# manycore-research/faceformer

Measured on AMD Instinct MI355X. Metric: decoded edges/sec (greedy face-loop decode, pointer selections/s), 256-edge wireframes, higher is better.
Workload: dtype f32; 1 GPU; BASELINE config 2: configs/ours.yml model.num_lines=256: 1 synthetic 256-edge wireframe(s) per GPU, F=256 anchor sequences x 36 greedy steps, default-xavier synthetic weights; wireframes_per_gpu=1, edges=256, max_face_length=37, decode_steps=36, parallelism=wireframe-sharded x1, RCCL all-gather of predictions

## Files before the change

faceformer_amd/csrc/ff_common.h:

```cpp
#pragma once
#include <hip/hip_runtime.h>
#include <stdint.h>
#include <stdio.h>
#include <string.h>

#include "faceformer_hip.h"

#define FF_WAVE 64
#define FF_MAX_STREAMS 8

typedef float f32x4 __attribute__((ext_vector_type(4)));
typedef float f32x16 __attribute__((ext_vector_type(16)));

void ff_set_error(const char* fmt, ...);

#define FF_CHECK_ARG(cond, ...)           \
  do {                                    \
    if (!(cond)) {                        \
      ff_set_error(__VA_ARGS__);          \
      return FF_ERR_ARG;                  \
    }                                     \
  } while (0)

#define FF_CHECK_HIP(expr)                                                             \
// ... 31 lines not shown
  ~FFProfScope() {
    if (on) ff_prof_close(st);
  }
};

unsigned long long ff_tuning_epoch();
void ff_tuning_changed();

int ff_num_cus();

enum FFKnob {
  FF_K_L0_FOLD = 0,
  FF_K_POINTER_FOLD,
  FF_K_LAST_QKV_ONE_LAUNCH_ROWS,
  FF_K_PINNED_COUNTERS,
  FF_K_DEBUG_TIMING,
  FF_K_DMA_MIN_ROWS, FF_K_DMA_MIN_ROWS_N512, FF_K_DMA_MIN_ROWS_WIDE,
  FF_K_SK_HYBRID, FF_K_SK_HYBRID_FIX, FF_K_SK_HYBRID_MAXLEFT8, FF_K_SK_HYBRID_MINU, FF_K_SK_HYBRID_FORCE,
  FF_K_NO_PANEL,
  FF_K_X3_SMALL_SPLIT,
  FF_K_RK_SPLIT_OLD, FF_K_RK_SPLIT_YOUNG, FF_K_RK_PHASE, FF_K_RK_ROTATE,
  FF_K_X3_NEED_N1024, FF_K_X3_NEED_N512,
  FF_K_X2H_ATTN,
  FF_K_COUNT
};
int ff_knob(int id);

size_t ff_attention_planes_stride();
bool ff_attention_x2h_ok(const ff_attn_desc& d);
int ff_attention_x2h_launch(const ff_attn_desc& d, const void* planes, long long plane_stride, hipStream_t st);

struct ff_pointer_sync {
  int* seen;
  int* arrive;
  int* host_slot;
  int host_which;
  float* next_stats;
  int logits_ready;
  const int* slot;
  int* fin;
  int fin_j, term_lo, term_hi;
};
int ff_pointer_argmax_sync(const float* p, int ldp, const float* memory, int S, int E, const unsigned char* mask,
                           const int* kv_len, const unsigned char* extra_mask, int ldextra, int B, int seqs_per_group,
                           int* next_tok, float* best, float* second, float* logprob, float* logits, int ldlogits,
                           float* next_rows, int ldnext, int* count_ge, int ge_bound, int* count_eq, int eq_value,
// ... 34 lines not shown
int ff_pointer_constrained_ahead_sync(float* logits, int ldlogits, int S, const unsigned char* mask, const int* kv_len, int B,
                                      int seqs_per_group, const unsigned* follows, int L, int flags, int ntok, int term_lo,
                                      int term_hi, const int* fin_in, const int* first_in, const int* prev_in, unsigned* visited,
                                      unsigned char* mask_rows, int* next_tok, float* logprob, int* fin_out, int* dead_end,
                                      int* first_out, int* prev_out, const float* memory, int E, float* next_rows, int ldnext,
                                      float* next_stats, int* count_ge, const unsigned char* close_dist,
                                      const unsigned char* cycle_len, int budget, int* arrive, int* host_slot, ff_stream_t stream);
int ff_constrain_init(int* tok, float* lp, int* fin, int* dead, int* first, int* prev, unsigned* visited, int Bc, int Fc, int f0,
                      const int* num_input, int pad_tok, int term_lo, int term_hi, int ntok, const unsigned* follows, int L,
                      hipStream_t st);
int ff_constrain_finalize(const int* tok, const float* lp, const int* fin, const int* dead, int Btot, int T, const int* steps_dev,
                          const int* num_input, int dedup, int F, int w0, int nw, int Fc, int f0, int b0, int64_t* predict,
                          float* logprob, int* dead_end, int* seq_of_row, hipStream_t st);

int ff_beam_constrained_select_sync(const ff_beam_constrained_step* step, int* arrive, int* host_slot, ff_stream_t stream);
int ff_constrain_beam_init(int* tok, float* score, int* fin, int* dead, int* parent, int* first, int* prev, unsigned* visited, int Bc,
                           int Fc, int W, int f0, const int* num_input, int pad_tok, int term_lo, int term_hi, int ntok,
                           const unsigned* follows, int L, hipStream_t st);
int ff_constrain_beam_dead(const int* dead, int Btot, const int* steps_dev, const int* num_input, int dedup, int F, int W, int w0,
                           int nw, int Fc, int f0, int b0, int* dead_end, hipStream_t st);

int ff_transpose(const float* in, int ld_in, int rows, int cols, float* out, int ld_out, hipStream_t st);

extern "C" __attribute__((visibility("hidden"))) int ff_x3_prepare_stream(hipStream_t st);
int ff_stream_scratch(hipStream_t st, size_t bytes, float** out);

__device__ __forceinline__ float ff_wave_sum(float v) {
#pragma unroll
  for (int off = 32; off > 0; off >>= 1) v += __shfl_xor(v, off, FF_WAVE);
  return v;
}
__device__ __forceinline__ float ff_wave_max(float v) {
#pragma unroll
  for (int off = 32; off > 0; off >>= 1) v = fmaxf(v, __shfl_xor(v, off, FF_WAVE));
  return v;
}

__device__ __forceinline__ float ff_halves_sum(float v) {
  const auto r = __builtin_amdgcn_permlane32_swap(__float_as_uint(v), __float_as_uint(v), false, false);
  return __uint_as_float(r[0]) + __uint_as_float(r[1]);
}
__device__ __forceinline__ float ff_halves_max(float v) {
  const auto r = __builtin_amdgcn_permlane32_swap(__float_as_uint(v), __float_as_uint(v), false, false);
  return fmaxf(__uint_as_float(r[0]), __uint_as_float(r[1]));
}

// ... 8 lines not shown
```

faceformer_amd/csrc/ff_device.h:

```cpp
#pragma once
#include "ff_common.h"

typedef float f32x2 __attribute__((ext_vector_type(2)));

#define FF_GLOBAL __attribute__((address_space(1)))
typedef unsigned long long ff_u64;

__device__ __forceinline__ f32x4 ff_ld16(const float* p) { return *reinterpret_cast<const f32x4*>(p); }
__device__ __forceinline__ f32x2 ff_ld8(const float* p) { return *reinterpret_cast<const f32x2*>(p); }
__device__ __forceinline__ float ff_ld4(const float* p) { return *p; }
__device__ __forceinline__ void ff_st16(float* p, f32x4 v) { *reinterpret_cast<f32x4*>(p) = v; }
__device__ __forceinline__ void ff_st8(float* p, f32x2 v) { *reinterpret_cast<f32x2*>(p) = v; }
__device__ __forceinline__ void ff_st4(float* p, float v) { *p = v; }
__device__ __forceinline__ int ff_ld4i(const int* p) { return *p; }
__device__ __forceinline__ void ff_st4i(int* p, int v) { *p = v; }
__device__ __forceinline__ void ff_store_tile(float* cp, int ldc, int row0, int col, int M, bool colok, const float (&v)[16]) {
  float* p = cp + (size_t)row0 * ldc + col;
  if (row0 - (row0 & 4) + 32 <= M) {
    if (colok) {
#pragma unroll
      for (int e = 0; e < 16; ++e) ff_st4(p + (size_t)((e & 3) + 8 * (e >> 2)) * ldc, v[e]);
    }
  } else {
#pragma unroll
// ... 14 lines not shown
  const float* res;
  float* C;
  int lda, ldw, ldr, ldc;
  int M, N, K;
  int n_split, act;
  int tiles_m, tiles_n;
  long long batch_stride_a, batch_stride_w, batch_stride_c;
  const float* ln_in;
  int ln_nseg;
  float ln_eps;
  const float* rowtab;
  int ld_rowtab, rowtab_div, rowtab_cols;
  float* ln_out;
};

bool ff_gemm_dma_f32_ok(const GemmArgs& a, int batch);
int ff_gemm_dma_f32(const GemmArgs& a, hipStream_t st, int bn = 128);

__device__ __forceinline__ float ff_sum8(float v) {
  v += __builtin_bit_cast(float, __builtin_amdgcn_update_dpp(0, __builtin_bit_cast(int, v), 0xB1, 0xF, 0xF, true));
  v += __builtin_bit_cast(float, __builtin_amdgcn_update_dpp(0, __builtin_bit_cast(int, v), 0x4E, 0xF, 0xF, true));
  v += __builtin_bit_cast(float, __builtin_amdgcn_update_dpp(0, __builtin_bit_cast(int, v), 0x141, 0xF, 0xF, true));
  return v;
}

__host__ __device__ constexpr int ff_gemm_small_lds_floats(int mode, int nw) {
  return nw * 16 * 64 + (mode == 2 ? 32 * 33 : 0) + (mode == 1 ? 64 : 0);
}

template <int KQ, int MODE, int NW>
__device__ __forceinline__ void ff_gemm_small_tile(const GemmArgs& g, int tile, long long bz, float* red) {
  static_assert(NW == 4 || NW == 8, "4 or 8 waves");
  constexpr int RPW = 16 / NW;
  const int tid = threadIdx.x, wave = tid >> 6, lane = tid & 63, half = lane >> 5, l32 = lane & 31;
  const int m0 = (tile / g.tiles_n) * 32, n0 = (tile % g.tiles_n) * 32;
  const float* Asrc = ((g.A2 != nullptr && n0 >= g.n_split) ? g.A2 : g.A) + bz * g.batch_stride_a;
  int row = m0 + l32, col = n0 + l32;
  row = row < g.M ? row : g.M - 1;
  col = col < g.N ? col : g.N - 1;
  const float* ap = Asrc + (size_t)row * g.lda + wave * KQ + half * 4;
  const float* wp = g.W + bz * g.batch_stride_w + (size_t)col * g.ldw + wave * KQ + half * 4;
  constexpr int NG = KQ / 8;
  constexpr int GB = NG < 4 ? NG : 4;
  f32x4 a[2][GB], b[2][GB];
#pragma unroll
  for (int j = 0; j < GB; ++j) {
// ... 709 lines not shown
```

faceformer_amd/csrc/ff_engine.hip:

```cpp
#include <chrono>
#include <cstdlib>
#include <mutex>
#include <vector>

#include "ff_common.h"
#include "ff_device.h"
#include "ff_launch.h"

namespace {

struct Bump {
  char* base;
  size_t size, off;
  bool ok;
  Bump(void* p, size_t n) : base((char*)p), size(n), off(0), ok(true) {}
  template <typename T>
  T* take(size_t count) {
    size_t bytes = ff_align_up(count * sizeof(T), 256);
    if (off + bytes > size) { ok = false; off += bytes; return nullptr; }
    T* r = reinterpret_cast<T*>(base + off);
    off += bytes;
    return r;
  }
};
// ... 112 lines not shown
    return gemm(d.A, d.lda, d.A2, d.n_split, d.W, d.ldw, d.bias, d.res, d.ldr, d.C, d.ldc, d.M, d.N, d.K, d.act, st);
  }
  ff_gemm_ln_desc g;
  memset(&g, 0, sizeof(g));
  g.A = d.A; g.lda = d.lda; g.W = d.W; g.ldw = d.ldw; g.bias = d.bias; g.residual = d.res; g.ldr = d.ldr; g.C = d.C; g.ldc = d.ldc;
  g.M = d.M; g.N = d.N; g.K = d.K; g.act = d.act; g.tile = 0;
  g.ln_stats_in = d.st_in; g.ln_nseg = d.K / 32; g.ln_eps = m->ln_eps;
  g.row_table = d.table; g.ld_row_table = d.ldt; g.row_div = row_div; g.row_cols = d.tcols;
  g.ln_stats_out = d.st_out;
  if (split) return sk.ln(&g, d.planes, d.plane_rows, d.row0, d.st_in ? d.colsum : nullptr, st);
  return ff_gemm_f32_ln(&g, st);
}

struct Scratch {
  float *x, *y, *yq, *qkv, *o, *h, *p, *logits;
  float* lnstat;
};

struct DecodeBuffers {
  float *mem_pos, *kvc[FF_MAX_LAYERS];
  unsigned char* kvp[FF_MAX_LAYERS];
  float *x0_all, *qkv0_all;
  float* x0stat_all;
  float *projT, *pg_all, *pc_all;
  int* tok_all;
  float* lp_all;
  Scratch scr[FF_MAX_STREAMS];
  int* zeroed; size_t zeroed_count;
  int *cnt_ge, *cnt_eq;
  int *arrive;
  int *seen;
  int *cnt_tot;
  int *steps_dev;
  int *fin, *slot_all, *perm_all;
  float* bm_score;
  int *bm_fin, *bm_parent;
  float* fc_lp;
  int *fc_greedy, *fc_rank;
  float* sm_lp;
  int *sm_fin, *sm_row;
  float* cn_lp;
  int *cn_fin, *cn_dead, *cn_first, *cn_prev;
  unsigned* cn_visited;
  unsigned char* cn_rows;
  int *cb_dead, *cb_first, *cb_prev;
  unsigned* cb_visited;
// ... 88 lines not shown
  const ff_constrain_beam_params* cbeam() const { return static_cast<const ff_constrain_beam_params*>(prm); }
};

void plan_mode(const ff_decode_params* p, const int* num_input_host, int ns, const Mode& mode, std::vector<Chunk>* out, int* btot,
               int* max_bc, int* nchunks = nullptr) {
  switch (mode.kind) {
    case Mode::BEAM:
    case Mode::CONSTRAIN_BEAM:
    case Mode::SAMPLE: return plan_beam_chunks(p, num_input_host, ns, mode.G, out, btot, max_bc, nchunks);
    case Mode::FORCED: {
      ff_decode_params q = *p;
      q.flags &= ~FF_DEDUP_PAD_ANCHORS;
      return plan_chunks(&q, nullptr, ns, out, btot, max_bc, nchunks);
    }
    default: return plan_chunks(p, num_input_host, ns, out, btot, max_bc, nchunks);
  }
}

constexpr int FF_PINNED_SLOTS = 65536;
struct EngineKnobs {
  bool l0_fold, pointer_fold, dbg_timing;
  bool x2h_attn;
  int one_launch_rows, pinned;
};
EngineKnobs engine_knobs(const ff_decode_params* p) {
  EngineKnobs k;
  k.l0_fold = ff_knob(FF_K_L0_FOLD) != 0 && !(p->flags & FF_NO_L0_FOLD);
  k.pointer_fold = ff_knob(FF_K_POINTER_FOLD) != 0 && !(p->flags & FF_NO_POINTER_FOLD);
  k.dbg_timing = ff_knob(FF_K_DEBUG_TIMING) != 0;
  k.x2h_attn = ff_knob(FF_K_X2H_ATTN) != 0;
  k.one_launch_rows = ff_knob(FF_K_LAST_QKV_ONE_LAUNCH_ROWS);
  const int pc = ff_knob(FF_K_PINNED_COUNTERS);
  k.pinned = pc > 0 && pc < FF_PINNED_SLOTS ? pc : FF_PINNED_SLOTS;
  return k;
}

bool can_fuse_layernorm(const ff_model* m, const ff_decode_params* prm) {
  if (!(prm->flags & FF_FUSE_LAYERNORM)) return false;
  if (m->E % 64 != 0 || m->E < 128 || m->E > 512 || m->FF % 64 != 0 || m->FF < 128) return false;
  if (!m->proj_fold_w || !m->proj_fold_b) return false;
  for (int l = 0; l < m->num_dec_layers; ++l) {
    const ff_layer_weights& w = m->dec[l];
    if (!w.ln1_w || !w.ln1_b || !w.ln1_pos || !w.ln2_w || !w.ln2_b || !w.ln2_pos || !w.ln3_w || !w.ln3_b) return false;
  }
  return true;
}

size_t layout_decode(const ff_model* m, const ff_decode_params* p, const EngineKnobs& kn, size_t Btot, size_t Bch, size_t nch,
                     Bump& bp, DecodeBuffers* out, const Mode& mode, bool want_lp = false) {
  const int E = m->E, FFd = m->FF, S = p->L + m->num_token, T = p->T;
  const int ns = plan_streams(p);
  const size_t Rmax = (size_t)(T - 1 > 0 ? T - 1 : 1) * Bch;
  DecodeBuffers b;
  memset(&b, 0, sizeof(b));
  b.mem_pos = bp.take<float>((size_t)p->N * S * E);
  for (int l = 0; l < m->num_dec_layers; ++l) b.kvc[l] = bp.take<float>((size_t)p->N * S * 2 * E);
  const bool planes = kn.x2h_attn && (m->split_kind == 1 || m->split_kind == 2) && p->x3_min_rows > 0 && S <= 288 && m->dec[0].in_proj_planes != nullptr;
  for (int l = 0; l < m->num_dec_layers; ++l)
    b.kvp[l] = planes ? bp.take<unsigned char>(ff_attention_planes_bytes(p->N, m->H)) : nullptr;
  b.x0_all = bp.take<float>((size_t)T * Btot * E);
  b.tok_all = bp.take<int>((size_t)T * Btot);
  b.qkv0_all = (p->flags & FF_REUSE_LAYER0_QKV) ? bp.take<float>((size_t)T * Btot * 3 * E) : nullptr;
  b.x0stat_all = (kn.l0_fold && (p->flags & FF_REUSE_LAYER0_QKV) && can_fuse_layernorm(m, p)) ? bp.take<float>(Btot * (size_t)(E / 32) * 2)
                                                                                 : nullptr;
  const bool pf = kn.pointer_fold && can_fuse_layernorm(m, p);
  b.projT = pf ? bp.take<float>((size_t)E * E) : nullptr;
  b.pg_all = pf ? bp.take<float>(nch * (size_t)S * E) : nullptr;
  b.pc_all = pf ? bp.take<float>(nch * (size_t)((S + 3) & ~3)) : nullptr;
  for (int s = 0; s < ns; ++s) {
    Scratch& c = b.scr[s];
    c.x = bp.take<float>(Rmax * E);
    c.y = bp.take<float>(Rmax * E);
    c.yq = bp.take<float>(Rmax * E);
    c.qkv = bp.take<float>(Rmax * 3 * E);
    c.o = bp.take<float>(Rmax * E);
    c.h = bp.take<float>(Rmax * FFd);
    c.p = bp.take<float>(Bch * E);
    c.logits = bp.take<float>(Bch * (size_t)S);
    c.lnstat = bp.take<float>(Rmax * (size_t)(E / 32 + 1) * 2);
  }
  const size_t ncnt = ff_align_up((size_t)T * nch * sizeof(int), 256) / sizeof(int);
  b.zeroed_count = 3 * ncnt + Btot;
  b.zeroed = bp.take<int>(b.zeroed_count);
  if (b.zeroed) { b.cnt_ge = b.zeroed; b.cnt_eq = b.cnt_ge + ncnt; b.arrive = b.cnt_eq + ncnt; b.seen = b.arrive + ncnt; }
  b.cnt_tot = bp.take<int>(T);
  b.steps_dev = bp.take<int>(4);
  if (retiring(p)) {
    b.fin = bp.take<int>(Btot);
    b.slot_all = bp.take<int>(Btot);
// ... 68 lines not shown
  return can_fuse_layernorm(m, prm) && R <= fuse_max;
}

int decoder_pass(const ff_model* m, const ff_decode_params* prm, const EngineKnobs& kn, const DecodeBuffers& bufs, const Scratch& buf,
                 const Chunk& ck, int Fc, int Bc, const unsigned char* mask, const int* kv_len, int t, bool full_rows,
                 float* proj_all, hipStream_t st, float* logits_out = nullptr) {
  const int E = m->E, FFd = m->FF, H = m->H, S = prm->L + m->num_token, F = Fc, T = prm->T;
  const int R = t * Bc, nd = m->num_dec_layers;
  const size_t newoff = (size_t)(t - 1) * Bc;
  const bool reuse0 = (prm->flags & FF_REUSE_LAYER0_QKV) != 0 && ck.qkv0 != nullptr;
  const bool prune_last = (prm->flags & FF_LAST_LAYER_LAST_ROW) != 0 && !full_rows;
  const bool fuse = step_fuses(m, prm, R);
  const int nseg = E / 32;
  const float* qpos = m->qpos_table;
  const float* qpos_new = qpos + (size_t)(t - 1) * E;
  auto proj = [&](const Proj& d) -> int { return project(m, prm, Bc, st, d); };
  const bool last_qkv_one = R <= kn.one_launch_rows;
  for (int l = 0; l < nd; ++l) {
    const ff_layer_weights& w = m->dec[l];
    const ff_mha_weights& sa = w.self_attn;
    const bool last = prune_last && (l == nd - 1);
    const float* xin = (l == 0) ? ck.x0 : buf.x;
    const float* QKV = buf.qkv;
    if (l == 0 && reuse0) {
      if (full_rows) {
      } else if (fuse && t > 1 && ck.x0stat) {
        FF_RETURN_IF(proj(Proj().in(xin + newoff * E, E).weight(w.ln1_w, E, w.ln1_b).norm(ck.x0stat)
                              .pos(w.ln1_pos + (size_t)(t - 1) * 2 * E, 2 * E, 2 * E).out(ck.qkv0 + newoff * 3 * E, 3 * E, Bc, 3 * E, E)));
      } else {
        FF_RETURN_IF(ff_layernorm(xin + newoff * E, E, w.norm1_w, w.norm1_b, m->ln_eps, buf.y, E, buf.yq, E,
                                  qpos_new, E, Bc, 1, Bc, E, st));
        FF_RETURN_IF(proj(Proj().in(buf.yq, E, buf.y, 2 * E).weight(sa.in_proj_w, E, sa.in_proj_b)
                              .out(ck.qkv0 + newoff * 3 * E, 3 * E, Bc, 3 * E, E)));
      }
      QKV = ck.qkv0;
    } else if (fuse && l > 0) {
      const bool kv_only = last && t > 1 && !last_qkv_one;
      const int c0 = kv_only ? E : 0;
      FF_RETURN_IF(proj(Proj().in(buf.x, E).weight(w.ln1_w + (size_t)c0 * E, E, w.ln1_b + c0).split(w.ln1_planes, 3 * E, c0, w.ln1_csum)
                            .norm(buf.lnstat).pos(w.ln1_pos + c0, 2 * E, 2 * E - c0).out(buf.qkv + c0, 3 * E, R, 3 * E - c0, E)));
      if (kv_only)
        FF_RETURN_IF(proj(Proj().in(xin + newoff * E, E).weight(w.ln1_w, E, w.ln1_b).norm(buf.lnstat + newoff * nseg * 2)
                              .pos(w.ln1_pos + (size_t)(t - 1) * 2 * E, 2 * E, E).out(buf.qkv + newoff * 3 * E, 3 * E, Bc, E, E)));
    } else {
      FF_RETURN_IF(ff_layernorm(xin, E, w.norm1_w, w.norm1_b, m->ln_eps, buf.y, E, buf.yq, E, qpos, E, Bc, T, R, E, st));
      const bool x3_here = w.in_proj_planes && prm->x3_min_rows > 0 && R >= (long)prm->x3_min_rows;
      if (last && t > 1 && !x3_here && (E % 64) == 0) {
        FF_RETURN_IF(proj(Proj().in(buf.yq, E, buf.y, E).weight(sa.in_proj_w + (size_t)E * E, E, sa.in_proj_b + E)
                              .out(buf.qkv + E, 3 * E, R, 2 * E, E)));
        FF_RETURN_IF(proj(Proj().in(buf.yq + newoff * E, E).weight(sa.in_proj_w, E, sa.in_proj_b)
                              .out(buf.qkv + newoff * 3 * E, 3 * E, Bc, E, E)));
      } else {
        FF_RETURN_IF(proj(Proj().in(buf.yq, E, buf.y, 2 * E).weight(sa.in_proj_w, E, sa.in_proj_b).split(w.in_proj_planes, 3 * E)
                              .out(buf.qkv, 3 * E, R, 3 * E, E)));
      }
    }
    const size_t roff = last ? newoff : 0;
    const int Rl = last ? Bc : R;
    float* x = buf.x + roff * E;
    float* o = buf.o + roff * E;
    float* h = buf.h + roff * FFd;
    float* qc = buf.qkv + roff * E;
    float* stat = fuse ? buf.lnstat + roff * nseg * 2 : nullptr;
    {
      ff_attn_desc d;
      memset(&d, 0, sizeof(d));
      d.q = QKV + roff * 3 * E; d.k = QKV + E; d.v = QKV + 2 * E; d.o = o;
      d.ldq = d.ldk = d.ldv = 3 * E; d.ldo = E;
      d.num_groups = Bc; d.num_heads = H; d.scale = 0.125f;
      d.nq = last ? 1 : t; d.q_group_stride = 1; d.q_inner = 1; d.q_outer_stride = Bc;
      d.nk = t; d.k_group_stride = 1; d.k_stride = Bc;
      FF_RETURN_IF(ff_attention(&d, st));
    }
    FF_RETURN_IF(proj(Proj().in(o, E).weight(sa.out_w, E, sa.out_b).split(w.self_out_planes, E).add(xin + roff * E, E)
                          .out(x, E, Rl, E, E).stats(stat)));
    if (fuse) {
      FF_RETURN_IF(proj(Proj().in(x, E).weight(w.ln2_w, E, w.ln2_b).split(w.ln2_planes, E, 0, w.ln2_csum).norm(stat)
                            .pos(w.ln2_pos + (last ? (size_t)(t - 1) * E : 0), E, E).out(qc, E, Rl, E, E)));
    } else {
      if (last)
        FF_RETURN_IF(ff_layernorm(x, E, w.norm2_w, w.norm2_b, m->ln_eps, nullptr, 0, buf.yq + roff * E, E, qpos_new, E, Bc, 1, Rl, E, st));
      else
        FF_RETURN_IF(ff_layernorm(buf.x, E, w.norm2_w, w.norm2_b, m->ln_eps, nullptr, 0, buf.yq, E, qpos, E, Bc, T, Rl, E, st));
      FF_RETURN_IF(proj(Proj().in(buf.yq + roff * E, E).weight(w.cross_attn.in_proj_w, E, w.cross_attn.in_proj_b)
                            .split(w.cross_q_planes, E).out(qc, E, Rl, E, E)));
    }
    {
      ff_attn_desc d;
      memset(&d, 0, sizeof(d));
      d.q = qc; d.k = bufs.kvc[l] + (size_t)ck.w0 * S * 2 * E; d.v = d.k + E; d.o = o;
      d.ldq = d.ldo = E; d.ldk = d.ldv = 2 * E;
      d.num_groups = ck.nw; d.num_heads = H; d.scale = 0.125f;
      d.nq = last ? F : F * t; d.q_group_stride = F; d.q_inner = F; d.q_outer_stride = Bc;
      d.nk = S; d.k_group_stride = S; d.k_stride = 1;
      d.kv_len = kv_len + ck.w0; d.key_mask = mask + (size_t)ck.w0 * S; d.mask_stride = S;
      if (bufs.kvp[l] && step_splits(m, prm, R))
        d.kv_planes = bufs.kvp[l] + (size_t)ck.w0 * H * (ff_attention_planes_bytes(1, H) / H);
// ... 250 lines not shown
    const hipStream_t main_st = io.main_st;
    const int RS = N * S;
    FF_RETURN_IF(ff_add_pos(memory, E, m->pos_table, E, 1, S, buf.mem_pos, E, RS, E, main_st));
    for (int l = 0; l < m->num_dec_layers; ++l) {
      const ff_mha_weights& c = m->dec[l].cross_attn;
      FF_RETURN_IF(gemm(buf.mem_pos, E, memory, E, c.in_proj_w + (size_t)E * E, E, c.in_proj_b + E, nullptr, 0,
                        buf.kvc[l], 2 * E, RS, 2 * E, E, 0, main_st));
      if (buf.kvp[l])
        FF_RETURN_IF(ff_attention_split_kv(buf.kvc[l], buf.kvc[l] + E, 2 * E, 2 * E, N, m->H, S, S, 1, buf.kvp[l], main_st));
    }
    FF_CHECK_HIP(hipMemsetAsync(buf.zeroed, 0, sizeof(int) * buf.zeroed_count, main_st));
    if (retire) {
      int *st_slot = pool->stage, *st_fin = pool->stage + Btot;
      for (const Chunk& c : chunks) {
        const std::vector<int>& hs = hslot[(size_t)(&c - chunks.data())];
        if (!hs.empty()) memcpy(st_slot + c.b0, hs.data(), sizeof(int) * hs.size());
      }
      FF_CHECK_HIP(hipMemcpyAsync(buf.slot_all, st_slot, sizeof(int) * (size_t)Btot, hipMemcpyHostToDevice, main_st));
      if (!fin_host) {
        memcpy(st_fin, hfin.data(), sizeof(int) * (size_t)Btot);
        FF_CHECK_HIP(hipMemcpyAsync(buf.fin, st_fin, sizeof(int) * (size_t)Btot, hipMemcpyHostToDevice, main_st));
      }
    }
    FF_RETURN_IF(fork());
    bool any_pg = false;
    for (const Chunk& c : chunks) any_pg = any_pg || c.pg != nullptr;
    if (any_pg) {
      FF_RETURN_IF(ff_transpose(m->proj_fold_w, E, E, E, buf.projT, E, main_st));
      FF_RETURN_IF(fork());
      for (const Chunk& c : chunks) {
        if (!c.pg) continue;
        const float* mem_w = memory + (size_t)c.w0 * S * E;
        FF_RETURN_IF(gemm(mem_w, E, nullptr, 0, buf.projT, E, nullptr, nullptr, 0, c.pg, E, S, E, E, 0, sts[c.sid]));
        FF_RETURN_IF(gemm(mem_w, E, nullptr, 0, m->proj_fold_b, E, nullptr, nullptr, 0, c.pc, 1, S, 1, E, 0, sts[c.sid]));
      }
    }
    for (const Chunk& c : chunks) {
      if (mode.kind != Mode::GREEDY) {
        FF_RETURN_IF(init_state(c));
        FF_RETURN_IF(ff_gather_rows(memory + (size_t)c.w0 * S * E, S, E, buf.tok_all + c.b0, c.Bc, c.Fc, c.x0, E, sts[c.sid]));
        continue;
      }
      hipLaunchKernelGGL(init_tokens_kernel, dim3(ff_cdiv(c.Bc, 256)), dim3(256), 0, sts[c.sid], buf.tok_all + c.b0,
                         c.Bc, c.Fc, c.f0, io.num_input ? io.num_input + c.w0 : nullptr, p->variant, m->num_token - 1,
                         p->tok_sos, c.slot, c.perm, c.slot ? c.Bl : 0);
      FF_CHECK_LAUNCH();
// ... 656 lines not shown
```

faceformer_amd/csrc/ff_rowops.hip:

```cpp
#include <stdarg.h>
#include <stdlib.h>
#include <string.h>

#include <atomic>
#include <mutex>

#include "ff_common.h"
#include "ff_device.h"
#include "ff_launch.h"

static thread_local char g_ff_error[512] = "";

void ff_set_error(const char* fmt, ...) {
  va_list ap;
  va_start(ap, fmt);
  vsnprintf(g_ff_error, sizeof(g_ff_error), fmt, ap);
  va_end(ap);
}

int ff_num_cus() {
  static std::atomic<int> cached[FF_MAX_DEVICES] = {};
  int dev = 0;
  if (hipGetDevice(&dev) != hipSuccess || dev < 0 || dev >= FF_MAX_DEVICES) return 256;
  int n = cached[dev].load(std::memory_order_relaxed);
  if (n == 0) {
    if (hipDeviceGetAttribute(&n, hipDeviceAttributeMultiprocessorCount, dev) != hipSuccess || n <= 0) n = 256;
    cached[dev].store(n, std::memory_order_relaxed);
  }
  return n;
}

namespace {
struct KnobDef { const char* name; int def; bool presence; };
const KnobDef g_knob_defs[FF_K_COUNT] = {
    {"FF_L0_FOLD", 1, false}, {"FF_POINTER_FOLD", 1, false}, {"FF_LAST_QKV_ONE_LAUNCH_ROWS", 512, false},
    {"FF_PINNED_COUNTERS", 65536, false}, {"FF_DEBUG_TIMING", 0, true},
    {"FF_DMA_MIN_ROWS", 4096, false}, {"FF_DMA_MIN_ROWS_N512", 7680, false}, {"FF_DMA_MIN_ROWS_WIDE", 2560, false},
    {"FF_SK_HYBRID", 1, false}, {"FF_SK_HYBRID_FIX", 10, false}, {"FF_SK_HYBRID_MAXLEFT8", 4, false},
    {"FF_SK_HYBRID_MINU", 2, false}, {"FF_SK_HYBRID_FORCE", 0, false},
    {"FF_NO_PANEL", 0, true}, {"FF_X3_SMALL_SPLIT", 0, false},
    {"FF_RK_SPLIT_OLD", 1, false}, {"FF_RK_SPLIT_YOUNG", 1, false}, {"FF_RK_PHASE", 0, false}, {"FF_RK_ROTATE", 1, false},
    {"FF_X3_NEED_N1024", 7, false}, {"FF_X3_NEED_N512", 11, false}, {"FF_X2H_ATTN", 1, false},
};
std::atomic<int> g_knobs[FF_K_COUNT];
std::once_flag g_knobs_once;
void knobs_init() {
  std::call_once(g_knobs_once, [] {
    for (int i = 0; i < FF_K_COUNT; ++i) {
      const char* e = getenv(g_knob_defs[i].name);
      g_knobs[i].store(e ? (g_knob_defs[i].presence ? 1 : atoi(e)) : g_knob_defs[i].def, std::memory_order_relaxed);
    }
  });
}
int knob_index(const char* name) {
  if (!name) return -1;
  for (int i = 0; i < FF_K_COUNT; ++i)
    if (strcmp(name, g_knob_defs[i].name) == 0) return i;
  return -1;
}
}

int ff_knob(int id) {
  knobs_init();
  return g_knobs[id].load(std::memory_order_relaxed);
}
// ... 440 lines not shown
```

faceformer_amd/hip/build.py:

```python
import hashlib
import os
import shutil
import subprocess
import sys

HERE = os.path.dirname(os.path.abspath(__file__))
PKG = os.path.dirname(HERE)
ROOT = os.path.dirname(PKG)
CSRC = os.path.join(PKG, "csrc")
INCLUDE = os.path.join(ROOT, "include")
LIB_PATH = os.path.join(HERE, "libfaceformer_hip.so")
BUILD_DIR = os.path.join(HERE, "build")
ARCH = "gfx950"
SOURCES = ["ff_rowops.hip", "ff_gemm.hip", "ff_gemm_x3.hip", "ff_attention.hip", "ff_attention_x2h.hip", "ff_attention_general.hip", "ff_pointer.hip", "ff_beam.hip", "ff_forced.hip", "ff_sample.hip", "ff_constrain.hip", "ff_constrain_beam.hip", "ff_engine.hip"]
FLAGS = ["-O3", "-std=c++17", "-fPIC", "--offload-arch=" + ARCH, "-I" + INCLUDE, "-I" + CSRC,
         "-Wall", "-Wno-unused-function"]


def _hipcc():
    exe = shutil.which("hipcc") or "/opt/rocm/bin/hipcc"
    if not os.path.exists(exe):
        raise RuntimeError("hipcc not found: the HIP extension cannot be built on this machine")
    return exe


def _digest(paths, flags=None):
    h = hashlib.sha256()
    h.update(" ".join(FLAGS if flags is None else flags).encode())
    for p in paths:
        with open(p, "rb") as f:
            h.update(f.read())
    return h.hexdigest()


def build(force=False, verbose=False):
    return _build(BUILD_DIR, LIB_PATH, FLAGS, force, verbose)

# ... 35 lines not shown
```

faceformer_amd/hip/lib.py:

```python
import ctypes as C
import os

HERE = os.path.dirname(os.path.abspath(__file__))
LIB_PATH = os.environ.get("FF_HIP_LIB") or os.path.join(HERE, "libfaceformer_hip.so")

FF_MAX_LAYERS = 16
FF_HEAD_DIM = 64
FF_PARALLEL, FF_SEQ2SEQ = 0, 1
FF_REUSE_LAYER0_QKV, FF_LAST_LAYER_LAST_ROW, FF_RETURN_POINTER, FF_NO_STOP, FF_DEDUP_PAD_ANCHORS = 1, 2, 4, 8, 16
FF_FUSE_LAYERNORM = 32
FF_STOP_EACH_EOS = 512
FF_NO_L0_FOLD = 1024
FF_NO_POINTER_FOLD = 2048
FF_RETIRE_FINISHED = 4096
FF_ABI_VERSION = 105

fptr = C.c_void_p


class HipExtensionError(RuntimeError):
    pass


class AttnDesc(C.Structure):
# ... 164 lines not shown
                                      C.c_int, C.c_int, C.c_int, C.c_int, C.c_int, C.c_int, C.c_int,
                                      C.c_longlong, C.c_longlong, C.c_longlong, fptr]),
    "ff_gemm_f32_ln": (C.c_int, [C.POINTER(GemmLnDesc), fptr]),
    "ff_fold_layernorm_linear": (C.c_int, [fptr, C.c_int, C.c_int, C.c_int, fptr, fptr, fptr, fptr, C.c_int, C.c_int,
                                           C.c_int, fptr, fptr, fptr, fptr]),
    "ff_split_weight_bytes": (C.c_size_t, [C.c_int, C.c_int]),
    "ff_split_weight_bf16x3": (C.c_int, [fptr, C.c_int, C.c_int, C.c_int, fptr, fptr]),
    "ff_gemm_x3": (C.c_int, [fptr, C.c_int, fptr, C.c_int, fptr, fptr, fptr, C.c_int, fptr, C.c_int,
                             C.c_int, C.c_int, C.c_int, C.c_int, fptr]),
    "ff_gemm_x3_ln": (C.c_int, [C.POINTER(GemmLnDesc), fptr, C.c_int, C.c_int, fptr, fptr]),
    "ff_split_weight_fp16x2_bytes": (C.c_size_t, [C.c_int, C.c_int]),
    "ff_split_weight_fp16x2": (C.c_int, [fptr, C.c_int, C.c_int, C.c_int, fptr, fptr]),
    "ff_gemm_x2h": (C.c_int, [fptr, C.c_int, fptr, C.c_int, fptr, fptr, fptr, C.c_int, fptr, C.c_int,
                              C.c_int, C.c_int, C.c_int, C.c_int, fptr]),
    "ff_gemm_x2h_ln": (C.c_int, [C.POINTER(GemmLnDesc), fptr, C.c_int, C.c_int, fptr, fptr]),
    "ff_split_weight_fp16_bytes": (C.c_size_t, [C.c_int, C.c_int]),
    "ff_split_weight_fp16": (C.c_int, [fptr, C.c_int, C.c_int, C.c_int, fptr, fptr]),
    "ff_gemm_h1": (C.c_int, [fptr, C.c_int, fptr, C.c_int, fptr, fptr, fptr, C.c_int, fptr, C.c_int,
                             C.c_int, C.c_int, C.c_int, C.c_int, fptr]),
    "ff_gemm_h1_ln": (C.c_int, [C.POINTER(GemmLnDesc), fptr, C.c_int, C.c_int, fptr, fptr]),
    "ff_set_x3_tuning": (C.c_int, [C.c_int]),
    "ff_attention": (C.c_int, [C.POINTER(AttnDesc), fptr]),
    "ff_attention_general": (C.c_int, [C.POINTER(AttnGeneralDesc), fptr]),
    "ff_set_attention_algo": (C.c_int, [C.c_int]),
    "ff_attention_planes_bytes": (C.c_size_t, [C.c_int, C.c_int]),
    "ff_attention_split_kv": (C.c_int, [fptr, fptr, C.c_int, C.c_int, C.c_int, C.c_int, C.c_int, C.c_int, C.c_int, fptr, fptr]),
    "ff_set_tuning": (C.c_int, [C.c_char_p, C.c_int]),
    "ff_get_tuning": (C.c_int, [C.c_char_p, C.POINTER(C.c_int)]),
    "ff_reset_tuning": (C.c_int, []),
    "ff_set_gemm_tuning": (C.c_int, [C.c_int, C.c_int, C.c_int, C.c_int]),
    "ff_pointer_argmax": (C.c_int, [fptr, C.c_int, fptr, C.c_int, C.c_int, fptr, fptr, fptr, C.c_int,
                                    C.c_int, C.c_int, fptr, fptr, fptr, fptr, C.c_int, fptr, C.c_int,
                                    fptr, C.c_int, fptr, C.c_int, fptr]),
    "ff_pointer_argmax_lp": (C.c_int, [fptr, C.c_int, fptr, C.c_int, C.c_int, fptr, fptr, fptr, C.c_int,
                                       C.c_int, C.c_int, fptr, fptr, fptr, fptr, C.c_int, fptr, C.c_int,
                                       fptr, C.c_int, fptr, C.c_int, fptr, fptr]),
    "ff_permute_rows": (C.c_int, [fptr, C.c_int, fptr, fptr, C.c_int, fptr, C.c_int, C.c_int, C.c_int, fptr]),
    "ff_gather_rows": (C.c_int, [fptr, C.c_int, C.c_int, fptr, C.c_int, C.c_int, fptr, C.c_int, fptr]),
    "ff_assemble_embedding": (C.c_int, [fptr, C.c_int, fptr, C.c_int, C.c_int, C.c_int, C.c_int, fptr,
                                        fptr]),
    "ff_prepare_mask": (C.c_int, [fptr, C.c_int, C.c_int, C.c_int, fptr, fptr, fptr]),
    "ff_encode_workspace_bytes": (C.c_size_t, [C.POINTER(Model), C.c_int, C.c_int]),
    "ff_encode": (C.c_int, [C.POINTER(Model), fptr, fptr, fptr, C.c_int, C.c_int, fptr, fptr,
                            C.c_size_t, fptr]),
    "ff_decode_workspace_bytes": (C.c_size_t, [C.POINTER(Model), C.POINTER(DecodeParams), C.POINTER(C.c_int)]),
    "ff_decode": (C.c_int, [C.POINTER(Model), C.POINTER(DecodeParams), fptr, fptr, fptr, fptr,
# ... 96 lines not shown
```

faceformer_amd/hip/ops.py:

```python
import ctypes as C

import torch

from . import lib as _L


import functools


def _stream():
    return torch.cuda.current_stream().cuda_stream


def _on_tensor_device(fn):
    @functools.wraps(fn)
    def wrapper(*args, **kwargs):
        devs = {a.device for a in list(args) + list(kwargs.values()) if torch.is_tensor(a) and a.is_cuda}
        if len(devs) > 1:
            raise _L.HipExtensionError("%s: tensors on different devices %s" % (fn.__name__, sorted(map(str, devs))))
        if not devs:
            return fn(*args, **kwargs)
        with torch.cuda.device(next(iter(devs))):
            return fn(*args, **kwargs)
    return wrapper
# ... 234 lines not shown
        if m is None:
            continue
        if m.dtype == torch.bool and dt == torch.uint8:
            m = m.to(torch.uint8)
        _dev(m, name, dt)
        if m.dim() == 2:
            want = (nq, nk)
        elif m.dim() == 3:
            want = (num_groups * num_heads, nq, nk)
        else:
            raise ValueError("%s must be 2-D [nq, nk] or 3-D [num_groups*num_heads, nq, nk]" % name)
        if tuple(m.shape) != want:
            raise ValueError("%s must have shape %s, got %s" % (name, want, tuple(m.shape)))
        m = m.contiguous()
        keep.append(m)
        ld, bs = nk, (nq * nk if m.dim() == 3 else 0)
        if (d.attn_bias or d.attn_mask) and (d.attn_ld != ld or d.attn_batch_stride != bs):
            raise ValueError("attn_bias and attn_mask must both be 2-D or both 3-D")
        d.attn_ld, d.attn_batch_stride = ld, bs
        setattr(d, name, m.data_ptr())
    d.scale = float(head_dim) ** -0.5 if scale is None else scale
    _L.check(_L.load().ff_attention_general(C.byref(d), _stream()), "ff_attention_general")
    del keep
    return out


@_on_tensor_device
def pointer_argmax(p, memory, mask=None, kv_len=None, extra_mask=None, seqs_per_group=1,
                   want_logits=False, want_rows=False, counters=None, ge_bound=0, eq_value=0, want_logprob=False):
    p, ldp = _rows(p, "p")
    _dev(memory, "memory")
    if memory.dim() != 3 or not memory.is_contiguous():
        raise ValueError("memory must be a contiguous [N, S, E] tensor")
    B, E = p.shape
    S = memory.size(1)
    dev = p.device
    nxt = torch.empty(B, device=dev, dtype=torch.int32)
    best = torch.empty(B, device=dev, dtype=torch.float32)
    second = torch.empty(B, device=dev, dtype=torch.float32)
    logits = torch.empty((B, S), device=dev, dtype=torch.float32) if want_logits else None
    rows = torch.empty((B, E), device=dev, dtype=torch.float32) if want_rows else None
    if mask is not None:
        _dev(mask, "mask", torch.uint8)
    if kv_len is not None:
        _dev(kv_len, "kv_len", torch.int32)
    ldextra = 0
# ... 449 lines not shown
```

include/faceformer_hip.h:

```cpp
#ifndef FACEFORMER_HIP_H
#define FACEFORMER_HIP_H

#include <stddef.h>
#include <stdint.h>

#ifdef __cplusplus
extern "C" {
#endif

typedef void* ff_stream_t;

enum ff_status {
  FF_OK = 0,
  FF_ERR_ARG = -1,
  FF_ERR_LAUNCH = -2,
  FF_ERR_WORKSPACE = -3,
  FF_ERR_NO_DEVICE = -4
};

#define FF_HEAD_DIM 64
#define FF_MAX_LAYERS 16

#define FF_ABI_VERSION 105
int ff_version(void);
// ... 97 lines not shown
                          int k_group_stride, int k_stride, void* planes, ff_stream_t stream);

int ff_attention(const ff_attn_desc* desc, ff_stream_t stream);
int ff_set_attention_algo(int algo);

typedef struct ff_attn_general_desc {
  const float* q; const float* k; const float* v; float* o;
  int ldq, ldk, ldv, ldo;
  int num_groups, num_heads, head_dim;
  int nq;
  int q_group_stride, q_inner, q_outer_stride;
  int nk;
  int k_group_stride, k_stride;
  const int* kv_len;
  const unsigned char* key_mask; int mask_stride;
  int causal;
  const float* attn_bias;
  const unsigned char* attn_mask;
  int attn_ld;
  long long attn_batch_stride;
  float scale;
} ff_attn_general_desc;
int ff_attention_general(const ff_attn_general_desc* desc, ff_stream_t stream);

int ff_set_tuning(const char* name, int value);
int ff_get_tuning(const char* name, int* value);
int ff_reset_tuning(void);

int ff_pointer_argmax(const float* p, int ldp, const float* memory, int S, int E,
                      const unsigned char* mask, const int* kv_len,
                      const unsigned char* extra_mask, int ldextra,
                      int B, int seqs_per_group,
                      int* next_tok, float* best, float* second, float* logits, int ldlogits,
                      float* next_rows, int ldnext,
                      int* count_ge, int ge_bound, int* count_eq, int eq_value,
                      ff_stream_t stream);
int ff_pointer_argmax_lp(const float* p, int ldp, const float* memory, int S, int E,
                         const unsigned char* mask, const int* kv_len,
                         const unsigned char* extra_mask, int ldextra,
                         int B, int seqs_per_group,
                         int* next_tok, float* best, float* second, float* logits, int ldlogits,
                         float* next_rows, int ldnext,
                         int* count_ge, int ge_bound, int* count_eq, int eq_value,
                         float* logprob, ff_stream_t stream);

int ff_gather_rows(const float* memory, int S, int E, const int* tok, int B, int seqs_per_group,
// ... 255 lines not shown
```

Baseline: 158,200 edges/s.

## Fold last-layer self-attention K/V projections into query-side and post-attention GEMMs

Result: faster. 160,400 edges/s (median of 6 runs) (+1.4%).

```diff
diff --git a/faceformer_amd/csrc/ff_attention_fold.hip b/faceformer_amd/csrc/ff_attention_fold.hip
--- /dev/null
+++ b/faceformer_amd/csrc/ff_attention_fold.hip
@@ -0,0 +1,209 @@
+#include "ff_common.h"
+#include "ff_device.h"
+#include "ff_launch.h"
+
+namespace {
+
+constexpr int FOLD_THREADS = 512;
+constexpr int FOLD_WAVES = FOLD_THREADS / FF_WAVE;
+constexpr int FOLD_MAX_H = 8;
+constexpr int FOLD_MAX_V = 2;
+constexpr int FOLD_PB = 4;
+constexpr int FOLD_HPG = 2;
+constexpr int FOLD_MAX_SMALL_FLOATS = 12000;
+constexpr int FOLD_MAX_LDS_BYTES = 150 * 1024;
+
+struct FoldArgs {
+  const float* x;
+  const float* stats;
+  const float* qt;
+  float* u;
+  float eps, scale;
+  int Bc, t, E, H;
+  int stage;
+};
+
+__global__ __launch_bounds__(FOLD_THREADS) void attention_prefix_fold_kernel(FoldArgs a) {
+  extern __shared__ float fold_lds[];
+  const int tid = threadIdx.x, wave = tid >> 6, lane = tid & 63;
+  const int E = a.E, H = a.H, t = a.t, Bc = a.Bc, nv = E >> 2, nseg = E >> 5, W = E + t;
+  const size_t b = blockIdx.x;
+  float* mr = fold_lds;
+  float* sc = fold_lds + 2 * t;
+  float* inv = sc + H * t;
+  float* xs = fold_lds + (((2 + H) * t + H + 3) & ~3);
+  const float* qrow = a.qt + b * (size_t)H * W;
+
+  float qv[FOLD_MAX_H][FOLD_MAX_V][4];
+#pragma unroll
+  for (int h = 0; h < FOLD_MAX_H; ++h)
+#pragma unroll
+    for (int v = 0; v < FOLD_MAX_V; ++v) {
+      const int c4 = lane + 64 * v;
+      const bool ok = h < H && c4 < nv;
+#pragma unroll
+      for (int i = 0; i < 4; ++i) qv[h][v][i] = ok ? ff_ldw(qrow + (size_t)h * W + c4 * 4 + i) : 0.f;
+    }
+
+  const int spart = lane & 7;
+  const bool sok = 2 * spart < nseg;
+  for (int j0 = wave; j0 < t; j0 += FOLD_WAVES * FOLD_PB) {
+    f32x4 sv[FOLD_PB], xv[FOLD_PB][FOLD_MAX_V];
+#pragma unroll
+    for (int p = 0; p < FOLD_PB; ++p) {
+      const int j = j0 + FOLD_WAVES * p;
+      sv[p] = f32x4{0.f, 0.f, 0.f, 0.f};
+#pragma unroll
+      for (int v = 0; v < FOLD_MAX_V; ++v) xv[p][v] = f32x4{0.f, 0.f, 0.f, 0.f};
+      if (j < t) {
+        const size_t row = (size_t)j * Bc + b;
+        if (sok) sv[p] = ff_ld16(a.stats + (row * nseg + 2 * spart) * 2);
+#pragma unroll
+        for (int v = 0; v < FOLD_MAX_V; ++v)
+          if (lane + 64 * v < nv) xv[p][v] = ff_ld16(a.x + row * E + (lane + 64 * v) * 4);
+      }
+    }
+#pragma unroll
+    for (int p = 0; p < FOLD_PB; ++p) {
+      const int j = j0 + FOLD_WAVES * p;
+      if (j < t) {
+        const f32x2 mv = ff_ln_merge8(sv[p], spart, nseg);
+        const float mean = mv.x, rstd = 1.0f / sqrtf(mv.y + a.eps);
+#pragma unroll
+        for (int v = 0; v < FOLD_MAX_V; ++v) {
+          const int c4 = lane + 64 * v;
+          xv[p][v] = c4 < nv ? (xv[p][v] - mean) * rstd : f32x4{0.f, 0.f, 0.f, 0.f};
+          if (a.stage && c4 < nv) ff_st16(xs + (size_t)j * E + c4 * 4, xv[p][v]);
+        }
+        if (lane == 0) { mr[2 * j] = mean; mr[2 * j + 1] = rstd; }
+#pragma unroll
+        for (int h = 0; h < FOLD_MAX_H; ++h) {
+          if (h < H) {
+            float s = 0.f;
+#pragma unroll
+            for (int v = 0; v < FOLD_MAX_V; ++v)
+#pragma unroll
+              for (int i = 0; i < 4; ++i) s += qv[h][v][i] * xv[p][v][i];
+            s = ff_wave_sum(s);
+            if (lane == 0) sc[h * t + j] = a.scale * (s + ff_ldw(qrow + (size_t)h * W + E + j));
+          }
+        }
+      }
+    }
+  }
+  __syncthreads();
+
+  for (int h = wave; h < H; h += FOLD_WAVES) {
+    float* s = sc + h * t;
+    float mx = -3.402823466e38f;
+    for (int j = lane; j < t; j += FF_WAVE) mx = fmaxf(mx, s[j]);
+    mx = ff_wave_max(mx);
+    float sum = 0.f;
+    for (int j = lane; j < t; j += FF_WAVE) {
+      const float e = expf(s[j] - mx);
+      s[j] = e;
+      sum += e;
+    }
+    sum = ff_wave_sum(sum);
+    if (lane == 0) inv[h] = 1.0f / sum;
+  }
+  __syncthreads();
+
+  const int groups = FOLD_THREADS / nv;
+  const int hpg = (H + groups - 1) / groups;
+  const int g = tid / nv, c4 = tid - g * nv, h0 = g * hpg;
+  if (g >= groups || h0 >= H) return;
+  f32x4 acc[FOLD_HPG];
+#pragma unroll
+  for (int k = 0; k < FOLD_HPG; ++k) acc[k] = f32x4{0.f, 0.f, 0.f, 0.f};
+  if (a.stage) {
+    const float* xc = xs + c4 * 4;
+#pragma unroll 4
+    for (int j = 0; j < t; ++j) {
+      const f32x4 xh = ff_ld16(xc + (size_t)j * E);
+#pragma unroll
+      for (int k = 0; k < FOLD_HPG; ++k)
+        if (k < hpg && h0 + k < H) acc[k] += sc[(h0 + k) * t + j] * xh;
+    }
+  } else {
+    const float* xc = a.x + b * E + c4 * 4;
+#pragma unroll 8
+    for (int j = 0; j < t; ++j) {
+      const f32x4 xh = (ff_ld16(xc + (size_t)j * Bc * E) - mr[2 * j]) * mr[2 * j + 1];
+#pragma unroll
+      for (int k = 0; k < FOLD_HPG; ++k)
+        if (k < hpg && h0 + k < H) acc[k] += sc[(h0 + k) * t + j] * xh;
+    }
+  }
+#pragma unroll
+  for (int k = 0; k < FOLD_HPG; ++k)
+    if (k < hpg && h0 + k < H) ff_st16(a.u + (b * H + (h0 + k)) * (size_t)E + c4 * 4, acc[k] * inv[h0 + k]);
+}
+
+__global__ __launch_bounds__(256) void attention_fold_tables_kernel(const float* __restrict__ w, const float* __restrict__ bias,
+                                                                    const float* __restrict__ pos, int pos_rows,
+                                                                    const float* __restrict__ out_w, const float* __restrict__ out_b,
+                                                                    int E, int H, int T, float* __restrict__ kt,
+                                                                    float* __restrict__ ob, int kt_blocks) {
+  const int tid = threadIdx.x;
+  if ((int)blockIdx.x < kt_blocks) {
+    const size_t i = (size_t)blockIdx.x * 256 + tid, total = (size_t)H * (E + T) * 64;
+    if (i >= total) return;
+    const int k = (int)(i & 63), n = (int)((i >> 6) % (size_t)(E + T)), h = (int)((i >> 6) / (size_t)(E + T));
+    const int c = E + 64 * h + k;
+    if (n < E) {
+      kt[i] = w[(size_t)c * E + n];
+    } else {
+      const int j = n - E < pos_rows ? n - E : pos_rows - 1;
+      kt[i] = bias[c] + pos[(size_t)j * 2 * E + c];
+    }
+    return;
+  }
+  const int n = ((int)blockIdx.x - kt_blocks) * 4 + (tid >> 6), lane = tid & 63;
+  if (n >= E) return;
+  float s = 0.f;
+  for (int k = lane; k < E; k += FF_WAVE) s += out_w[(size_t)n * E + k] * bias[2 * E + k];
+  s = ff_wave_sum(s);
+  if (lane == 0) ob[n] = out_b[n] + s;
+}
+
+}
+
+size_t ff_attention_fold_table_floats(int E, int H, int T) { return (size_t)H * (E + T) * 64 + (size_t)E; }
+
+int ff_attention_fold_tables(const float* ln1_w, const float* ln1_b, const float* ln1_pos, int pos_rows, const float* out_w,
+                             const float* out_b, int E, int H, int T, float* kt, float* ob, hipStream_t st) {
+  FF_CHECK_ARG(ln1_w && ln1_b && ln1_pos && out_w && out_b && kt && ob && pos_rows > 0 && T > 0 && E == H * FF_HEAD_DIM,
+               "ff_attention_fold_tables: bad arguments");
+  const size_t total = (size_t)H * (E + T) * 64;
+  const int kt_blocks = (int)((total + 255) / 256);
+  FFProfScope prof(FF_CAT_ROWOP, (double)total * 8.0, st);
+  hipLaunchKernelGGL(attention_fold_tables_kernel, dim3(kt_blocks + ff_cdiv(E, 4)), dim3(256), 0, st, ln1_w, ln1_b, ln1_pos,
+                     pos_rows, out_w, out_b, E, H, T, kt, ob, kt_blocks);
+  FF_CHECK_LAUNCH();
+  return FF_OK;
+}
+
+extern "C" int ff_attention_prefix_fold(const float* x, const float* stats, float ln_eps, const float* qt, float scale,
+                                        int Bc, int t, int E, int H, float* u, ff_stream_t stream) {
+  if (Bc == 0) return FF_OK;
+  FF_CHECK_ARG(x && stats && qt && u, "ff_attention_prefix_fold: null operand");
+  FF_CHECK_ARG(E % 64 == 0 && E >= 128 && E <= 512 && H == E / FF_HEAD_DIM,
+               "ff_attention_prefix_fold: needs E %% 64 == 0, 128 <= E <= 512 and H = E / 64 (E=%d H=%d)", E, H);
+  FF_CHECK_ARG(Bc > 0 && t > 0 && ln_eps >= 0.f, "ff_attention_prefix_fold: bad Bc=%d t=%d", Bc, t);
+  const long small_floats = (((long)(2 + H) * t + H + 3) & ~3L);
+  FF_CHECK_ARG(small_floats <= FOLD_MAX_SMALL_FLOATS, "ff_attention_prefix_fold: t=%d is past the %d score floats a block keeps", t,
+               FOLD_MAX_SMALL_FLOATS);
+  FF_CHECK_ARG(ff_aligned16(x) && ff_aligned16(stats) && ff_aligned16(u), "ff_attention_prefix_fold: x / stats / u must be 16-byte aligned");
+  const hipStream_t st = (hipStream_t)stream;
+  const long staged_bytes = (small_floats + (long)t * E) * (long)sizeof(float);
+  const int stage = staged_bytes <= FOLD_MAX_LDS_BYTES ? 1 : 0;
+  const size_t lds_bytes = stage ? (size_t)staged_bytes : (size_t)small_floats * sizeof(float);
+  static FFLdsLimit attr_set = {};
+  FF_RETURN_IF(ff_lds_limit_once(&attention_prefix_fold_kernel, FOLD_MAX_LDS_BYTES, &attr_set));
+  FoldArgs a{x, stats, qt, u, ln_eps, scale, Bc, t, E, H, stage};
+  FFProfScope prof(FF_CAT_ATTN, 4.0 * Bc * (double)t * H * E, st);
+  hipLaunchKernelGGL(attention_prefix_fold_kernel, dim3(Bc), dim3(FOLD_THREADS), lds_bytes, st, a);
+  FF_CHECK_LAUNCH();
+  return FF_OK;
+}
diff --git a/faceformer_amd/csrc/ff_common.h b/faceformer_amd/csrc/ff_common.h
--- a/faceformer_amd/csrc/ff_common.h
+++ b/faceformer_amd/csrc/ff_common.h
@@ -77,6 +77,7 @@
   FF_K_RK_SPLIT_OLD, FF_K_RK_SPLIT_YOUNG, FF_K_RK_PHASE, FF_K_RK_ROTATE,
   FF_K_X3_NEED_N1024, FF_K_X3_NEED_N512,
   FF_K_X2H_ATTN,
+  FF_K_LAST_FOLD_MIN_ROWS,
   FF_K_COUNT
 };
 int ff_knob(int id);
@@ -157,6 +158,10 @@
 
 int ff_transpose(const float* in, int ld_in, int rows, int cols, float* out, int ld_out, hipStream_t st);
 
+size_t ff_attention_fold_table_floats(int E, int H, int T);
+int ff_attention_fold_tables(const float* ln1_w, const float* ln1_b, const float* ln1_pos, int pos_rows, const float* out_w,
+                             const float* out_b, int E, int H, int T, float* kt, float* ob, hipStream_t st);
+
 extern "C" __attribute__((visibility("hidden"))) int ff_x3_prepare_stream(hipStream_t st);
 int ff_stream_scratch(hipStream_t st, size_t bytes, float** out);
 
diff --git a/faceformer_amd/csrc/ff_device.h b/faceformer_amd/csrc/ff_device.h
--- a/faceformer_amd/csrc/ff_device.h
+++ b/faceformer_amd/csrc/ff_device.h
@@ -60,6 +60,17 @@
   v += __builtin_bit_cast(float, __builtin_amdgcn_update_dpp(0, __builtin_bit_cast(int, v), 0x4E, 0xF, 0xF, true));
   v += __builtin_bit_cast(float, __builtin_amdgcn_update_dpp(0, __builtin_bit_cast(int, v), 0x141, 0xF, 0xF, true));
   return v;
+}
+
+__device__ __forceinline__ f32x2 ff_ln_merge8(const f32x4& sv, int spart, int nseg) {
+  const bool sok = 2 * spart < nseg;
+  const float fn = (float)nseg;
+  const float mean = ff_sum8(sok ? sv.x + sv.z : 0.f) / fn;
+  const float m2 = ff_sum8(sok ? sv.y + sv.w : 0.f);
+  const float d0 = sv.x - mean, d1 = sv.z - mean;
+  const float dev = ff_sum8(sok ? d0 * d0 + d1 * d1 : 0.f);
+  const float var = (m2 + 32.f * dev) / (32.f * fn);
+  return f32x2{mean, var};
 }
 
 __host__ __device__ constexpr int ff_gemm_small_lds_floats(int mode, int nw) {
diff --git a/faceformer_amd/csrc/ff_engine.hip b/faceformer_amd/csrc/ff_engine.hip
--- a/faceformer_amd/csrc/ff_engine.hip
+++ b/faceformer_amd/csrc/ff_engine.hip
@@ -158,6 +158,7 @@
   unsigned char* kvp[FF_MAX_LAYERS];
   float *x0_all, *qkv0_all;
   float* x0stat_all;
+  float *fold_kt, *fold_ob;
   float *projT, *pg_all, *pc_all;
   int* tok_all;
   float* lp_all;
@@ -292,6 +293,7 @@
   bool l0_fold, pointer_fold, dbg_timing;
   bool x2h_attn;
   int one_launch_rows, pinned;
+  int last_fold_rows;
 };
 EngineKnobs engine_knobs(const ff_decode_params* p) {
   EngineKnobs k;
@@ -300,6 +302,7 @@
   k.dbg_timing = ff_knob(FF_K_DEBUG_TIMING) != 0;
   k.x2h_attn = ff_knob(FF_K_X2H_ATTN) != 0;
   k.one_launch_rows = ff_knob(FF_K_LAST_QKV_ONE_LAUNCH_ROWS);
+  k.last_fold_rows = ff_knob(FF_K_LAST_FOLD_MIN_ROWS);
   const int pc = ff_knob(FF_K_PINNED_COUNTERS);
   k.pinned = pc > 0 && pc < FF_PINNED_SLOTS ? pc : FF_PINNED_SLOTS;
   return k;
@@ -335,6 +338,9 @@
                                                                                  : nullptr;
   const bool pf = kn.pointer_fold && can_fuse_layernorm(m, p);
   b.projT = pf ? bp.take<float>((size_t)E * E) : nullptr;
+  const bool lf = kn.last_fold_rows > 0 && Rmax >= (size_t)kn.last_fold_rows && (p->flags & FF_LAST_LAYER_LAST_ROW) && m->num_dec_layers > 1 && can_fuse_layernorm(m, p);
+  b.fold_kt = lf ? bp.take<float>(ff_attention_fold_table_floats(E, m->H, T)) : nullptr;
+  b.fold_ob = b.fold_kt ? b.fold_kt + (size_t)m->H * (E + T) * 64 : nullptr;
   b.pg_all = pf ? bp.take<float>(nch * (size_t)S * E) : nullptr;
   b.pc_all = pf ? bp.take<float>(nch * (size_t)((S + 3) & ~3)) : nullptr;
   for (int s = 0; s < ns; ++s) {
@@ -449,6 +455,7 @@
     const bool last = prune_last && (l == nd - 1);
     const float* xin = (l == 0) ? ck.x0 : buf.x;
     const float* QKV = buf.qkv;
+    bool fold_last = false;
     if (l == 0 && reuse0) {
       if (full_rows) {
       } else if (fuse && t > 1 && ck.x0stat) {
@@ -462,13 +469,28 @@
       }
       QKV = ck.qkv0;
     } else if (fuse && l > 0) {
+      const size_t qt_floats = ff_align_up((size_t)Bc * H * (E + t), 4);
+      fold_last = last && t > 1 && bufs.fold_kt && R >= kn.last_fold_rows && !step_splits(m, prm, R) &&
+                  qt_floats + (size_t)Bc * H * E <= (size_t)(T - 1 > 0 ? T - 1 : 1) * Bc * FFd;
       const bool kv_only = last && t > 1 && !last_qkv_one;
       const int c0 = kv_only ? E : 0;
-      FF_RETURN_IF(proj(Proj().in(buf.x, E).weight(w.ln1_w + (size_t)c0 * E, E, w.ln1_b + c0).split(w.ln1_planes, 3 * E, c0, w.ln1_csum)
-                            .norm(buf.lnstat).pos(w.ln1_pos + c0, 2 * E, 2 * E - c0).out(buf.qkv + c0, 3 * E, R, 3 * E - c0, E)));
-      if (kv_only)
+      if (!fold_last)
+        FF_RETURN_IF(proj(Proj().in(buf.x, E).weight(w.ln1_w + (size_t)c0 * E, E, w.ln1_b + c0).split(w.ln1_planes, 3 * E, c0, w.ln1_csum)
+                              .norm(buf.lnstat).pos(w.ln1_pos + c0, 2 * E, 2 * E - c0).out(buf.qkv + c0, 3 * E, R, 3 * E - c0, E)));
+      if (kv_only || fold_last)
         FF_RETURN_IF(proj(Proj().in(xin + newoff * E, E).weight(w.ln1_w, E, w.ln1_b).norm(buf.lnstat + newoff * nseg * 2)
                               .pos(w.ln1_pos + (size_t)(t - 1) * 2 * E, 2 * E, E).out(buf.qkv + newoff * 3 * E, 3 * E, Bc, E, E)));
+      if (fold_last) {
+        float* qt = buf.h;
+        float* u = buf.h + qt_floats;
+        FF_RETURN_IF(ff_gemm_f32_batched(buf.qkv + newoff * 3 * E, 3 * E, nullptr, 0, bufs.fold_kt, FF_HEAD_DIM, nullptr, nullptr, 0,
+                                         qt, H * (E + t), Bc, E + t, FF_HEAD_DIM, 0, 0, H, FF_HEAD_DIM,
+                                         (long long)(E + T) * FF_HEAD_DIM, E + t, st));
+        FF_RETURN_IF(ff_attention_prefix_fold(buf.x, buf.lnstat, m->ln_eps, qt, 0.125f, Bc, t, E, H, u, st));
+        FF_RETURN_IF(ff_gemm_f32_batched(u, H * E, nullptr, 0, w.ln1_w + (size_t)2 * E * E, E, nullptr, nullptr, 0,
+                                         buf.o + newoff * E, E, Bc, FF_HEAD_DIM, E, 0, 0, H, E, (long long)FF_HEAD_DIM * E,
+                                         FF_HEAD_DIM, st));
+      }
     } else {
       FF_RETURN_IF(ff_layernorm(xin, E, w.norm1_w, w.norm1_b, m->ln_eps, buf.y, E, buf.yq, E, qpos, E, Bc, T, R, E, st));
       const bool x3_here = w.in_proj_planes && prm->x3_min_rows > 0 && R >= (long)prm->x3_min_rows;
@@ -489,7 +511,7 @@
     float* h = buf.h + roff * FFd;
     float* qc = buf.qkv + roff * E;
     float* stat = fuse ? buf.lnstat + roff * nseg * 2 : nullptr;
-    {
+    if (!fold_last) {
       ff_attn_desc d;
       memset(&d, 0, sizeof(d));
       d.q = QKV + roff * 3 * E; d.k = QKV + E; d.v = QKV + 2 * E; d.o = o;
@@ -499,7 +521,7 @@
       d.nk = t; d.k_group_stride = 1; d.k_stride = Bc;
       FF_RETURN_IF(ff_attention(&d, st));
     }
-    FF_RETURN_IF(proj(Proj().in(o, E).weight(sa.out_w, E, sa.out_b).split(w.self_out_planes, E).add(xin + roff * E, E)
+    FF_RETURN_IF(proj(Proj().in(o, E).weight(sa.out_w, E, fold_last ? bufs.fold_ob : sa.out_b).split(w.self_out_planes, E).add(xin + roff * E, E)
                           .out(x, E, Rl, E, E).stats(stat)));
     if (fuse) {
       FF_RETURN_IF(proj(Proj().in(x, E).weight(w.ln2_w, E, w.ln2_b).split(w.ln2_planes, E, 0, w.ln2_csum).norm(stat)
@@ -796,6 +818,11 @@
         FF_CHECK_HIP(hipMemcpyAsync(buf.fin, st_fin, sizeof(int) * (size_t)Btot, hipMemcpyHostToDevice, main_st));
       }
     }
+    if (buf.fold_kt) {
+      const ff_layer_weights& w = m->dec[m->num_dec_layers - 1];
+      FF_RETURN_IF(ff_attention_fold_tables(w.ln1_w, w.ln1_b, w.ln1_pos, m->qpos_len, w.self_attn.out_w, w.self_attn.out_b, E, m->H, T,
+                                            buf.fold_kt, buf.fold_ob, main_st));
+    }
     FF_RETURN_IF(fork());
     bool any_pg = false;
     for (const Chunk& c : chunks) any_pg = any_pg || c.pg != nullptr;
diff --git a/faceformer_amd/csrc/ff_rowops.hip b/faceformer_amd/csrc/ff_rowops.hip
--- a/faceformer_amd/csrc/ff_rowops.hip
+++ b/faceformer_amd/csrc/ff_rowops.hip
@@ -41,6 +41,7 @@
     {"FF_NO_PANEL", 0, true}, {"FF_X3_SMALL_SPLIT", 0, false},
     {"FF_RK_SPLIT_OLD", 1, false}, {"FF_RK_SPLIT_YOUNG", 1, false}, {"FF_RK_PHASE", 0, false}, {"FF_RK_ROTATE", 1, false},
     {"FF_X3_NEED_N1024", 7, false}, {"FF_X3_NEED_N512", 11, false}, {"FF_X2H_ATTN", 1, false},
+    {"FF_LAST_FOLD_MIN_ROWS", 2048, false},
 };
 std::atomic<int> g_knobs[FF_K_COUNT];
 std::once_flag g_knobs_once;
diff --git a/faceformer_amd/hip/build.py b/faceformer_amd/hip/build.py
--- a/faceformer_amd/hip/build.py
+++ b/faceformer_amd/hip/build.py
@@ -12,7 +12,7 @@
 LIB_PATH = os.path.join(HERE, "libfaceformer_hip.so")
 BUILD_DIR = os.path.join(HERE, "build")
 ARCH = "gfx950"
-SOURCES = ["ff_rowops.hip", "ff_gemm.hip", "ff_gemm_x3.hip", "ff_attention.hip", "ff_attention_x2h.hip", "ff_attention_general.hip", "ff_pointer.hip", "ff_beam.hip", "ff_forced.hip", "ff_sample.hip", "ff_constrain.hip", "ff_constrain_beam.hip", "ff_engine.hip"]
+SOURCES = ["ff_rowops.hip", "ff_gemm.hip", "ff_gemm_x3.hip", "ff_attention.hip", "ff_attention_x2h.hip", "ff_attention_general.hip", "ff_attention_fold.hip", "ff_pointer.hip", "ff_beam.hip", "ff_forced.hip", "ff_sample.hip", "ff_constrain.hip", "ff_constrain_beam.hip", "ff_engine.hip"]
 FLAGS = ["-O3", "-std=c++17", "-fPIC", "--offload-arch=" + ARCH, "-I" + INCLUDE, "-I" + CSRC,
          "-Wall", "-Wno-unused-function"]
 
diff --git a/faceformer_amd/hip/lib.py b/faceformer_amd/hip/lib.py
--- a/faceformer_amd/hip/lib.py
+++ b/faceformer_amd/hip/lib.py
@@ -210,6 +210,7 @@
     "ff_set_x3_tuning": (C.c_int, [C.c_int]),
     "ff_attention": (C.c_int, [C.POINTER(AttnDesc), fptr]),
     "ff_attention_general": (C.c_int, [C.POINTER(AttnGeneralDesc), fptr]),
+    "ff_attention_prefix_fold": (C.c_int, [fptr, fptr, C.c_float, fptr, C.c_float, C.c_int, C.c_int, C.c_int, C.c_int, fptr, fptr]),
     "ff_set_attention_algo": (C.c_int, [C.c_int]),
     "ff_attention_planes_bytes": (C.c_size_t, [C.c_int, C.c_int]),
     "ff_attention_split_kv": (C.c_int, [fptr, fptr, C.c_int, C.c_int, C.c_int, C.c_int, C.c_int, C.c_int, C.c_int, fptr, fptr]),
diff --git a/faceformer_amd/hip/ops.py b/faceformer_amd/hip/ops.py
--- a/faceformer_amd/hip/ops.py
+++ b/faceformer_amd/hip/ops.py
@@ -280,6 +280,20 @@
     d.scale = float(head_dim) ** -0.5 if scale is None else scale
     _L.check(_L.load().ff_attention_general(C.byref(d), _stream()), "ff_attention_general")
     del keep
+    return out
+
+
+@_on_tensor_device
+def attention_prefix_fold(x, stats, qt, Bc, t, E, H, eps=1e-5, scale=0.125, out=None):
+    _dev(x, "x"), _dev(stats, "stats"), _dev(qt, "qt")
+    for name, a in (("x", x), ("stats", stats), ("qt", qt)):
+        if not a.is_contiguous():
+            raise ValueError("attention_prefix_fold: %s must be contiguous" % name)
+    if out is None:
+        out = torch.empty((Bc, H * E), device=x.device, dtype=torch.float32)
+    _dev(out, "out")
+    _L.check(_L.load().ff_attention_prefix_fold(_p(x), _p(stats), eps, _p(qt), scale, Bc, t, E, H, _p(out), _stream()),
+             "ff_attention_prefix_fold")
     return out
 
 
diff --git a/include/faceformer_hip.h b/include/faceformer_hip.h
--- a/include/faceformer_hip.h
+++ b/include/faceformer_hip.h
@@ -143,6 +143,9 @@
   float scale;
 } ff_attn_general_desc;
 int ff_attention_general(const ff_attn_general_desc* desc, ff_stream_t stream);
+
+int ff_attention_prefix_fold(const float* x, const float* stats, float ln_eps, const float* qt, float scale,
+                             int Bc, int t, int E, int H, float* u, ff_stream_t stream);
 
 int ff_set_tuning(const char* name, int value);
 int ff_get_tuning(const char* name, int* value);
```
